# kaist-ina/BWA-MEME

Hardware: AMD Instinct MI355X
Metric: seeding_reads_per_sec (higher is better)
Workload: dtype u64; 1 GPU; learned-index seeding (rounds 1-3 + hit gather), 150 bp SE reads vs 3100 Mbp synthetic genome (fwd+rc suffix array of 6200000000 entries), index and reads resident in HBM; genome_bp=3100000000, sa_entries=6200000000, read_len=150, rmi_leaves_log2=28

## Files before the change

bwa-meme_amd/csrc/meme_seed.hip:

```cpp
#include <limits.h>
#include <stdlib.h>
#include <string.h>
#include <utility>

#include "meme_seed_kernel.h"

namespace {

using namespace seedk;

constexpr int SCAN_BLOCK = 256;
constexpr int SCAN_ITEMS = 4;
constexpr int SCAN_TILE = SCAN_BLOCK * SCAN_ITEMS;

__device__ __forceinline__ i64 block_scan_excl(i64 v, i64* total) {
    __shared__ i64 wsum[SCAN_BLOCK / 64];
    const int lane = threadIdx.x & 63, wid = threadIdx.x >> 6;
    i64 x = v;
#pragma unroll
    for (int d = 1; d < 64; d <<= 1) {
        i64 y = __shfl_up(x, d);
        if (lane >= d) x += y;
    }
    if (lane == 63) wsum[wid] = x;
// ... 103 lines not shown
            if (hits_per_smem > 0 && h > hits_per_smem) h = hits_per_smem;
            i64 incl = h;
#pragma unroll
            for (int d = 1; d < GL; d <<= 1) {
                i64 y = __shfl_up(incl, d, GL);
                if (t >= d) incl += y;
            }
            const i64 hb = hb0 + incl - h;
            u64 first = 0;
            if (act) {
                first = (s.sa_start & SLOT_POS) ? (u64)(s.sa_start & SLOT_VAL) : sa[s.sa_start].pos;
                meme_mem_tl m;
                m.start = s.start;
                m.end = s.end;
                m.hitbeg = (int32_t)hb;
                m.hitcount = s.count > (i64)INT_MAX ? INT_MAX : (int32_t)s.count;
                m.cache_refpos = first;
                out[k] = m;
                if (h > 0) hout[hb] = first;
                for (i64 i = 1; i < h && i < 4; ++i) hout[hb + i] = sa[s.sa_start + i].pos;
            }
            u64 longmask = (__ballot(act && h > 4) >> gbase) & 0xffffull;
            while (longmask) {
                const int src = __ffsll((long long)longmask) - 1;
                longmask &= longmask - 1;
                const i64 lh = __shfl(h, src, GL), lhb = __shfl(hb, src, GL), lsa = __shfl(s.sa_start, src, GL);
                for (i64 i = 4 + t; i < lh; i += GL) hout[lhb + i] = sa[lsa + i].pos;
            }
            hb0 += __shfl(incl, GL - 1, GL);
        }
    }
}

template <int G>
int launch_k_seed(hipStream_t stream, const SeedArgs& A, size_t lds, i64 blocks) {
    if (lds > 64 * 1024)
        HIP_TRY(hipFuncSetAttribute((const void*)k_seed<G>, hipFuncAttributeMaxDynamicSharedMemorySize, (int)lds));
    hipLaunchKernelGGL(k_seed<G>, dim3((unsigned)blocks), dim3(BLOCK), lds, stream, A);
    HIP_TRY(hipGetLastError());
    return MEME_OK;
}

struct SeedRun {
    meme_ctx* ctx;
    const i64* d_read_off; i64 nreads;
    const meme_seed_opt* opt;
    PackGeom geo;
    TierTable tiers = {};
    bool defer = false;
    i64 n_early = -1;
    i64 n_todo = 0;
    float ms_total = 0.f, ms_reseed = 0.f;
    i64 launches = 0, searches = 0, windows = 0, lane_searches = 0;
};

int seed_pack(SeedRun& R, const uint8_t* d_reads, i64 max_len, i64 total_bytes) {
    meme_ctx* ctx = R.ctx;
    if (max_len > MAX_READ_LEN) {
        meme_set_error("read of %lld bases exceeds the learned-index limit of %d (LEARNED_MAX_READ_LEN)", (long long)max_len, MAX_READ_LEN);
        return MEME_E_ARG;
    }
    if (max_len < 1) max_len = 1;
    PackGeom& geo = R.geo;
    geo.W = (int)((max_len + 31) / 32) + 2;
    geo.MW = (int)((max_len + 63) / 64);
    geo.stride = 2 * geo.W + 2 * geo.MW + 1;
    int rc;
    if ((rc = meme_buf_reserve(ctx, ctx->batch.packed, (size_t)R.nreads * geo.stride * 8))) return rc;
    HIP_TRY(hipEventRecord(ctx->seed.ev[SEED_EV_PACK0], ctx->stream));
    int rb = (int)((48 * 1024) / max_len);
    if (rb > 32) rb = 32;
    if (rb < 1) rb = 1;
    i64 pblocks = (R.nreads + rb - 1) / rb;
    if (pblocks > (i64)ctx->n_cus * 16) pblocks = (i64)ctx->n_cus * 16;
    size_t plds = ((size_t)rb * (size_t)max_len + 16 + 48 + 3) & ~(size_t)3;
    hipLaunchKernelGGL(k_pack_reads, dim3((unsigned)pblocks), dim3(256), plds, ctx->stream, d_reads,
                       R.d_read_off, R.nreads, total_bytes, geo, rb, (u64*)ctx->batch.packed.p);
    HIP_TRY(hipGetLastError());
    HIP_TRY(hipEventRecord(ctx->seed.ev[SEED_EV_PACK1], ctx->stream));
    return MEME_OK;
}

int launch_tier(SeedRun& R, int tier, i64 n_todo, const i64* pending, int cset, hipStream_t stream, bool defer) {
    meme_ctx* ctx = R.ctx;
    int G = tier == 0 ? (int)ctx->group_lanes : 32;
    const int cap = tier == 0 ? (int)ctx->smem_cap : TIER_CAP[tier];
    const int lcap = cap < TIER_LCAP[tier] ? cap : TIER_LCAP[tier];
    DevBuf& sb = ctx->seed.slots[tier];
    DevBuf& ob = ctx->seed.ovf[tier & 1];
    const size_t need = (size_t)n_todo * cap * sizeof(SlotRec);
    if (tier > 0 && need > sb.cap) {
        size_t free_b = 0;
        if (!meme_fits_free_hbm(need, 0, &free_b)) {
            meme_set_error("%lld reads emitted more than %d SMEMs each: re-running them needs %.1f GB of slots, more than half of the "
                           "free HBM (%.1f GB); seed this batch in smaller pieces", (long long)n_todo, R.tiers.cap[tier - 1],
                           need / 1e9, free_b / 1e9);
            return MEME_E_CAPACITY;
        }
    }
    int rc;
    if ((rc = meme_buf_reserve(ctx, sb, need))) return rc;
    if ((rc = meme_buf_reserve(ctx, ob, (size_t)n_todo * sizeof(i64)))) return rc;
    unsigned long long* counters = ctx->seed.counter_set(cset);
    HIP_TRY(hipMemsetAsync(counters, 0, SEED_CTRS * sizeof(unsigned long long), stream));
    SeedArgs A;
    A.I = ctx->idx;
    A.packed = (const u64*)ctx->batch.packed.p;
    A.read_off = R.d_read_off;
    A.nreads = n_todo;
    A.geo = R.geo;
    A.opt = *R.opt;
    A.slots = (SlotRec*)sb.p;
    A.slot_cnt = (int*)ctx->seed.slot_cnt.p;
    A.slot_hits = (i64*)ctx->seed.slot_hits.p;
    A.slot_loc = (i64*)ctx->seed.slot_loc.p;
    A.pending = pending;
    A.ovf_list = (i64*)ob.p;
    A.cap = cap;
    A.lcap = lcap;
    A.tier = tier;
    A.counters = counters;
    A.defer = defer ? 1 : 0;
    R.tiers.base[tier] = (const SlotRec*)sb.p;
    R.tiers.cap[tier] = cap;
    while (G < 32 && seed_lds_bytes(G, R.geo, lcap) > (size_t)160 * 1024) G *= 2;
    const int groups = BLOCK / G;
    size_t lds = seed_lds_bytes(G, R.geo, lcap);
    i64 want = (n_todo + groups - 1) / groups;
    i64 blocks = ctx->seed_blocks > 0 ? ctx->seed_blocks : (i64)ctx->n_cus * ctx->seed_blocks_per_cu;
    if (blocks > want) blocks = want;
    if (blocks < 1) blocks = 1;
    if (tier == 0) HIP_TRY(hipEventRecord(ctx->seed.ev[SEED_EV_SEARCH0], stream));
    switch (G) {
    case 1: return launch_k_seed<1>(stream, A, lds, blocks);
    case 2: return launch_k_seed<2>(stream, A, lds, blocks);
    case 4: return launch_k_seed<4>(stream, A, lds, blocks);
    case 8: return launch_k_seed<8>(stream, A, lds, blocks);
    case 16: return launch_k_seed<16>(stream, A, lds, blocks);
    case 32: return launch_k_seed<32>(stream, A, lds, blocks);
    default: meme_set_error("group_lanes must be 1, 2, 4, 8, 16 or 32"); return MEME_E_ARG;
    }
}

int fetch_counters(SeedRun& R, int cset, unsigned long long* h) {
    HIP_TRY(hipMemcpyAsync(h, R.ctx->seed.counter_set(cset), SEED_CTRS * sizeof(unsigned long long), hipMemcpyDeviceToHost, R.ctx->stream));
    HIP_TRY(hipStreamSynchronize(R.ctx->stream));
    return MEME_OK;
}
void tally(SeedRun& R, const unsigned long long* h) {
    ++R.launches;
    R.searches += (i64)h[SEED_CTR_SEARCHES];
    R.windows += (i64)h[SEED_CTR_WINDOWS];
    R.n_todo = (i64)h[SEED_CTR_OVERFLOW];
#ifdef SEED_PROF
    {
        double tot = 0; for (int k = 0; k < 8; ++k) tot += (double)h[SEED_CTR_PROF + k];
        fprintf(stderr, "[seed prof]:");
        const char* nm[6] = {"control", "request+rmi", "window+compare", "resolve", "level", "apply"};
        for (int k = 0; k < 6; ++k) fprintf(stderr, " %s %.1f%%", nm[k], 100.0 * (double)h[SEED_CTR_PROF + k] / (tot > 0 ? tot : 1));
        fprintf(stderr, "\n");
    }
#endif
}

int launch_reseed(SeedRun& R) {
    meme_ctx* ctx = R.ctx;
    SeedWs& S = ctx->seed;
    const i64 nreads = R.nreads;
    HIP_TRY(hipEventRecord(S.ev[SEED_EV_RESEED0], ctx->stream));
    ReseedArgs A;
    A.I = ctx->idx; A.packed = (const u64*)ctx->batch.packed.p; A.geo = R.geo; A.nreads = nreads; A.opt = *R.opt;
    A.slots = (SlotRec*)S.slots[0].p; A.cap = (int)ctx->smem_cap; A.slot_cnt = (int*)S.slot_cnt.p; A.slot_hits = (i64*)S.slot_hits.p;
    A.ovf_list = (i64*)S.ovf[0].p; A.counters = S.counter_set(0); A.pend_list = (i64*)S.pend.p;
    A.blk = (BlkRec*)S.blk.p; A.blk_out = A.blk + nreads * BLK_PER_READ; A.blk_cap = nreads * BLK_PER_READ;
    A.blk_ctr = SEED_CTR_BLK; A.blk_out_ctr = SEED_CTR_BLK_OUT;
    i64 rblocks = (nreads + 255) / 256;
    if (rblocks > (i64)ctx->n_cus * 32) rblocks = (i64)ctx->n_cus * 32;
    hipLaunchKernelGGL(k_reseed, dim3((unsigned)rblocks), dim3(256), 0, ctx->stream, A);
    HIP_TRY(hipEventRecord(ctx->side.fork[0], ctx->stream));
    const unsigned sblocks = (unsigned)(rblocks < (i64)ctx->n_cus * 4 ? rblocks : (i64)ctx->n_cus * 4);
    if (!S.emit.s) HIP_TRY(hipStreamCreateWithFlags(&S.emit.s, hipStreamNonBlocking));
    for (int i = 0; i < 2; ++i) if (!S.emit_ev[i]) HIP_TRY(hipEventCreateWithFlags(&S.emit_ev[i], hipEventDisableTiming));
    HIP_TRY(hipEventRecord(S.emit_ev[0], ctx->stream));
    HIP_TRY(hipStreamWaitEvent(S.emit, S.emit_ev[0], 0));
    hipLaunchKernelGGL(k_reseed_emit, dim3(sblocks), dim3(256), 0, S.emit, A);
    HIP_TRY(hipEventRecord(S.emit_ev[1], S.emit));
    constexpr int ROUNDS = 4;
    for (int round = 0; round < ROUNDS; ++round) {
        hipLaunchKernelGGL(k_reseed_search, dim3(sblocks), dim3(256), 0, ctx->stream, A);
        if (round < ROUNDS - 1) {
            hipLaunchKernelGGL(k_reseed_resume<false>, dim3(sblocks), dim3(256), 0, ctx->stream, A);
            HIP_TRY(hipMemsetAsync(S.counter_set(0) + A.blk_ctr, 0, sizeof(unsigned long long), ctx->stream));
            std::swap(A.blk, A.blk_out); std::swap(A.blk_ctr, A.blk_out_ctr);
        } else hipLaunchKernelGGL(k_reseed_resume<true>, dim3(sblocks), dim3(256), 0, ctx->stream, A);
    }
    HIP_TRY(hipGetLastError());
    return MEME_OK;
}

int launch_early_overflow(SeedRun& R) {
    meme_ctx* ctx = R.ctx;
    Stream& side = ctx->side.st[0];
    unsigned long long h_ovf = 0;
    HIP_TRY(hipStreamWaitEvent(side, ctx->side.fork[0], 0));
    HIP_TRY(hipMemcpyAsync(&h_ovf, ctx->seed.counter_set(0) + SEED_CTR_OVERFLOW, 8, hipMemcpyDeviceToHost, side));
    HIP_TRY(hipStreamSynchronize(side));
    if (h_ovf == 0) return MEME_OK;
    R.n_early = (i64)h_ovf;
    int rc;
    if ((rc = launch_tier(R, 1, R.n_early, (const i64*)ctx->seed.ovf[0].p, 1, side, false))) return rc;
    HIP_TRY(hipEventRecord(ctx->side.done[0], side));
    HIP_TRY(hipStreamWaitEvent(ctx->stream, ctx->side.done[0], 0));
    return MEME_OK;
}

int seed_tier0(SeedRun& R) {
    meme_ctx* ctx = R.ctx;
    SeedWs& S = ctx->seed;
    int rc;
    R.defer = ctx->seed_defer != 0 && ctx->idx.plcp != nullptr && R.opt->rounds >= 2;
    if (R.defer && (rc = meme_buf_reserve(ctx, S.pend, (size_t)R.nreads * sizeof(i64)))) return rc;
    if (R.defer && (rc = meme_buf_reserve(ctx, S.blk, (size_t)R.nreads * BLK_PER_READ * 2 * sizeof(BlkRec)))) return rc;
    if ((rc = launch_tier(R, 0, R.nreads, nullptr, 0, ctx->stream, R.defer))) return rc;
    if (R.defer) {
        if ((rc = meme_side_stream(ctx, 0)) || (rc = launch_reseed(R)) || (rc = launch_early_overflow(R))) return rc;
        HIP_TRY(hipStreamWaitEvent(ctx->stream, S.emit_ev[1], 0));
    }
    HIP_TRY(hipEventRecord(S.ev[SEED_EV_SEARCH1], ctx->stream));
    unsigned long long h[SEED_CTRS];
    if ((rc = fetch_counters(R, 0, h))) return rc;
    float ms = 0.f;
    HIP_TRY(hipEventElapsedTime(&ms, S.ev[SEED_EV_SEARCH0], S.ev[SEED_EV_SEARCH1]));
    R.ms_total += ms;
    if (R.defer) {
        float a = 0.f;
        HIP_TRY(hipEventElapsedTime(&a, S.ev[SEED_EV_RESEED0], S.ev[SEED_EV_SEARCH1]));
        R.ms_reseed += a;
        R.lane_searches += (i64)h[SEED_CTR_LANE];
        if (getenv("MEME_SEED_TRACE")) fprintf(stderr, "[meme] seed tier 0: search kernel + re-seeding kernels %.2f ms, of which behind k_seed %.2f ms (%lld lane searches; %lld reads of the "
                                               "overflow tier beside them)\n", ms, a, (long long)h[SEED_CTR_LANE], (long long)(R.n_early < 0 ? 0 : R.n_early));
    }
    tally(R, h);
    return MEME_OK;
}

int seed_overflow_tiers(SeedRun& R) {
    meme_ctx* ctx = R.ctx;
    SeedWs& S = ctx->seed;
    int rc;
    unsigned long long h[SEED_CTRS];
    for (int tier = 1; R.n_todo > 0; ++tier) {
        if (tier >= N_TIERS) {
            meme_set_error("a read produced more than %d SMEMs", TIER_CAP[N_TIERS - 1]);
            return MEME_E_CAPACITY;
        }
        const int cset = tier & 1;
        if (tier == 1 && R.n_early == R.n_todo) {
            if ((rc = fetch_counters(R, cset, h))) return rc;
        } else {
            HIP_TRY(hipEventRecord(S.ev[SEED_EV_SEARCH0], ctx->stream));
            if ((rc = launch_tier(R, tier, R.n_todo, (const i64*)S.ovf[(tier - 1) & 1].p, cset, ctx->stream, false))) return rc;
            HIP_TRY(hipEventRecord(S.ev[SEED_EV_SEARCH1], ctx->stream));
            if ((rc = fetch_counters(R, cset, h))) return rc;
            float ms = 0.f;
            HIP_TRY(hipEventElapsedTime(&ms, S.ev[SEED_EV_SEARCH0], S.ev[SEED_EV_SEARCH1]));
            R.ms_total += ms;
        }
        tally(R, h);
    }
    return MEME_OK;
}

int seed_gather(SeedRun& R, meme_seed_result* out) {
    meme_ctx* ctx = R.ctx;
    SeedWs& S = ctx->seed;
    ResidentBatch& B = ctx->batch;
    const i64 nreads = R.nreads;
    int rc;
    i64 ntiles = (nreads + SCAN_TILE - 1) / SCAN_TILE;
    if ((rc = meme_buf_reserve(ctx, ctx->scan_tmp, (size_t)(2 * ntiles + 2) * sizeof(i64)))) return rc;
    if ((rc = meme_buf_reserve(ctx, B.smem_off, (size_t)(nreads + 1) * sizeof(i64)))) return rc;
    if ((rc = meme_buf_reserve(ctx, B.hit_off, (size_t)(nreads + 1) * sizeof(i64)))) return rc;
    i64* tiles = (i64*)ctx->scan_tmp.p;
    i64* totals = tiles + 2 * ntiles;
    HIP_TRY(hipEventRecord(S.ev[SEED_EV_GATHER0], ctx->stream));
    hipLaunchKernelGGL(k_tile_sums, dim3((unsigned)ntiles), dim3(SCAN_BLOCK), 0, ctx->stream, (const int*)S.slot_cnt.p,
                       (const i64*)S.slot_hits.p, nreads, tiles);
    hipLaunchKernelGGL(k_scan_tiles, dim3(1), dim3(SCAN_BLOCK), 0, ctx->stream, tiles, ntiles, totals);
    hipLaunchKernelGGL(k_offsets, dim3((unsigned)ntiles), dim3(SCAN_BLOCK), 0, ctx->stream, (const int*)S.slot_cnt.p,
                       (const i64*)S.slot_hits.p, nreads, (const i64*)tiles, (i64*)B.smem_off.p, (i64*)B.hit_off.p);
    HIP_TRY(hipGetLastError());
    i64 h_tot[2];
    HIP_TRY(hipMemcpyAsync(h_tot, totals, sizeof(h_tot), hipMemcpyDeviceToHost, ctx->stream));
    HIP_TRY(hipStreamSynchronize(ctx->stream));
    if ((rc = meme_buf_reserve(ctx, B.smems, (size_t)(h_tot[0] + 1) * sizeof(meme_mem_tl)))) return rc;
    if ((rc = meme_buf_reserve(ctx, B.hits, (size_t)(h_tot[1] + 1) * sizeof(u64)))) return rc;
    i64 gblocks = (nreads + 15) / 16;
    if (gblocks > (i64)ctx->n_cus * 8) gblocks = (i64)ctx->n_cus * 8;
    if (gblocks < 1) gblocks = 1;
    hipLaunchKernelGGL(k_gather, dim3((unsigned)gblocks), dim3(BLOCK), 0, ctx->stream, ctx->idx.sa, R.tiers,
                       (const i64*)S.slot_loc.p, (const int*)S.slot_cnt.p, nreads, R.opt->hits_per_smem,
                       (const i64*)B.smem_off.p, (const i64*)B.hit_off.p, (meme_mem_tl*)B.smems.p, (u64*)B.hits.p);
    HIP_TRY(hipGetLastError());
    HIP_TRY(hipEventRecord(S.ev[SEED_EV_GATHER1], ctx->stream));
    HIP_TRY(hipStreamSynchronize(ctx->stream));
    HIP_TRY(hipEventElapsedTime(&ctx->tm.seed_gather_ms, S.ev[SEED_EV_GATHER0], S.ev[SEED_EV_GATHER1]));
    out->d_smems = (const meme_mem_tl*)B.smems.p;
    out->d_smem_off = (const i64*)B.smem_off.p;
    out->d_hits = (const u64*)B.hits.p;
    out->d_hit_off = (const i64*)B.hit_off.p;
    out->total_smems = h_tot[0];
// ... 250 lines not shown
```

bwa-meme_amd/csrc/meme_seed_kernel.h:

```cpp
#pragma once
#include <limits.h>

#include "meme_common.h"

namespace seedk {

constexpr int BLOCK = 256;
constexpr int MAX_READ_LEN = 500;

struct SlotRec {
    int32_t start, end;
    i64 sa_start;
    i64 count;
};
constexpr i64 SLOT_POS = 1ll << 62;
constexpr i64 SLOT_DEFER = 1ll << 61;
constexpr i64 SLOT_PEND = 1ll << 59;
constexpr i64 SLOT_VAL = (1ll << 48) - 1;
constexpr int DEFER_MAX_K = 64;


constexpr int N_TIERS = 3;
constexpr int TIER_CAP[N_TIERS] = {64, 2048, 65536};
#ifndef LCAP0
// ... 819 lines not shown


__device__ __forceinline__ u64 ext_g(const u64* __restrict__ w, int s) {
    const int k = s >> 5, sh = (s & 31) * 2;
    const u64 a = w[k], b = w[k + 1];
    return sh ? (a << sh) | (b >> (64 - sh)) : a;
}

struct LaneQuery {
    const u64* s;
    int off, vlen;
    u64 wq;
};

__device__ __forceinline__ void lane_compare_ent(const DevIndex& I, const LaneQuery& q, int cap, const SaEnt e, int& lcp, bool& less) {
    const i64 nlimit = I.n - (i64)cap;
    int Lc = cap;
    if ((i64)e.pos > nlimit) Lc = (int)(I.n - (i64)e.pos);
    const u64 x = e.key ^ q.wq;
    bool lt = e.key < q.wq;
    int l = x ? (__clzll((long long)x) >> 1) : 32;
    if (!x && 32 < Lc) {
        const i64 p0 = (i64)e.pos + 32;
        for (int k = 1;; ++k) {
            const u64 wr = extract32(I.pac, p0 + 32 * (k - 1));
            const u64 qq = ext_g(q.s, q.off + 32 * k);
            const u64 y = wr ^ qq;
            if (y) { l += __clzll((long long)y) >> 1; lt = wr < qq; break; }
            l += 32;
            if (l >= Lc) break;
        }
    }
    if (l >= Lc) { lcp = Lc; less = (i64)e.pos < nlimit; }
    else { lcp = l; less = lt; }
}
__device__ __forceinline__ void lane_compare(const DevIndex& I, const LaneQuery& q, int cap, i64 slot, int& lcp, bool& less) {
    lane_compare_ent(I, q, cap, I.sa[slot], lcp, less);
}

constexpr int LANE_W = 16;
struct LaneWin {
    uint32_t* lw;
    i64 base;
    __device__ __forceinline__ bool has(i64 slot) const { return base >= 0 && slot >= base && slot < base + LANE_W; }
    __device__ __forceinline__ int get(i64 slot) const { const int i = (int)(slot - base); return (int)((lw[(i >> 1) * 256] >> (16 * (i & 1))) & 0xffffu); }
};
__device__ __forceinline__ int lane_lcp(const DevIndex& I, const LaneQuery& q, const LaneWin& C, int cap, i64 slot) {
    if (C.has(slot)) return C.get(slot);
    int lc; bool ls;
    lane_compare(I, q, cap, slot, lc, ls);
    return lc;
}

__device__ __forceinline__ void lane_search(const DevIndex& I, const LaneQuery& q, int min_intv, uint32_t* lw, int& r_L, i64& r_start, i64& r_count) {
    const i64 n = I.n;
    u64 key = q.wq;
    if (q.vlen < 32) key |= (~0ull) >> (2 * q.vlen);
    u64 err;
    const i64 p = rmi_lookup((glb_rmi)I.l2, (glb_rmi)I.l1, I.n_l1, I.shift, n, key, err);
    LaneWin C; C.lw = lw; C.base = -1;
    int L = 0;
    i64 s = 0, e = 0;
    bool located = false;
    int lc; bool ls;
    {
        const i64 below = (i64)((err >> 32) & 0x3fffffffull) + 1, above = (i64)(err & 0x7fffffffull);
        const i64 span = below + above + 1;
        i64 base = span <= LANE_W ? p - below - (LANE_W - span) / 2 : p - (below * LANE_W) / span;
        if (base < 0) base = 0;
        if (base > n - LANE_W) base = n - LANE_W;
        SaEnt ent[LANE_W];
#pragma unroll
        for (int k = 0; k < LANE_W; ++k) ent[k] = I.sa[base + k];
        unsigned lessm = 0;
        int prev = 0;
#pragma unroll
        for (int k = 0; k < LANE_W; ++k) {
            lane_compare_ent(I, q, q.vlen, ent[k], lc, ls);
            lessm |= (ls ? 1u : 0u) << k;
            if (k & 1) lw[(k >> 1) * 256] = (uint32_t)prev | ((uint32_t)lc << 16); else prev = lc;
        }
        C.base = base;
        const int P = __popc(lessm);
        if (lessm == ((1u << P) - 1u) && ((P > 0 && P < LANE_W) || (P == 0 && base == 0) || (P == LANE_W && base + LANE_W == n))) {
            const int lm = P > 0 ? C.get(base + P - 1) : -1, lp = P < LANE_W ? C.get(base + P) : -1;
            L = lm >= lp ? lm : lp;
            s = e = base + (lm >= lp ? P - 1 : P);
            located = true;
        }
    }
    if (!located) {
        i64 lo = -1, hi = n;
        lane_compare(I, q, q.vlen, p, lc, ls);
        if (ls) {
            lo = p;
            for (i64 st = 1; hi == n && lo < n - 1; st <<= 1) {
                i64 pr = lo + st; if (pr > n - 1) pr = n - 1;
                lane_compare(I, q, q.vlen, pr, lc, ls);
                if (ls) lo = pr; else hi = pr;
            }
        } else {
            hi = p;
            for (i64 st = 1; lo == -1 && hi > 0; st <<= 1) {
                i64 pr = hi - st; if (pr < 0) pr = 0;
                lane_compare(I, q, q.vlen, pr, lc, ls);
                if (ls) lo = pr; else hi = pr;
            }
        }
        while (hi - lo > 1) {
            const i64 mid = lo + (hi - lo) / 2;
            lane_compare(I, q, q.vlen, mid, lc, ls);
            if (ls) lo = mid; else hi = mid;
        }
        const i64 P = hi;
        const int lm = P > 0 ? lane_lcp(I, q, C, q.vlen, P - 1) : -1, lp = P < n ? lane_lcp(I, q, C, q.vlen, P) : -1;
        L = lm >= lp ? lm : lp;
        s = e = lm >= lp ? P - 1 : P;
    }
    for (;;) {
        while (s > 0 && C.has(s - 1) && C.get(s - 1) >= L) --s;
        if (s > 0 && !C.has(s - 1)) {
            i64 good = s, bad = -1;
            for (i64 st = 1; good > 0; st <<= 1) {
                i64 pr = good - st; if (pr < 0) pr = 0;
                if (lane_lcp(I, q, C, L, pr) >= L) good = pr; else { bad = pr; break; }
            }
            while (bad >= 0 && good - bad > 1) {
                const i64 mid = bad + (good - bad) / 2;
                if (lane_lcp(I, q, C, L, mid) >= L) good = mid; else bad = mid;
            }
            s = good;
        }
        while (e < n - 1 && C.has(e + 1) && C.get(e + 1) >= L) ++e;
        if (e < n - 1 && !C.has(e + 1)) {
            i64 good = e, bad = n;
// ... 85 lines not shown
    }
};

struct RegionState { int pivot, next, guard, stage; };

template <bool OWNED>
__device__ __forceinline__ bool region_walk(const PlcpView& V, i64 n, i64 T0, int qbeg, int qend, int l_seq, int msl, RegionState& S, unsigned& hops,
                                            SmemAppender<OWNED>& ap, int& n_pend) {
    for (;;) {
        if (S.stage == 0) {
            const int plc = V.fwd(T0 + S.pivot);
            if (plc == 0 || plc == 255 || plc >= qend - S.pivot) return true;
            ++hops; S.next = S.pivot + plc; S.stage = 1;
        }
        if (S.stage == 1) {
            if (S.pivot >= S.next || ++S.guard > 4 * l_seq + 16) { S.stage = 3; return false; }
            const int plc = (S.pivot >= qbeg && S.pivot < qend) ? V.rev(n - 1 - (T0 + S.pivot)) : 0;
            if (plc == 0 || plc == 255 || plc >= S.pivot - qbeg + 1) return true;
            ++hops; S.pivot = S.pivot - plc + 1;
            if (S.next - S.pivot < msl) { S.stage = 3; return false; }
            S.stage = 2;
        }
        const int plc = (S.pivot >= qbeg && S.pivot < qend) ? V.fwd(T0 + S.pivot) : 0;
        if (plc == 0 || plc == 255 || plc >= qend - S.pivot) return true;
        if (plc >= msl) {
            if (!OWNED) return true;
            ap.push(S.pivot, S.pivot + plc, SLOT_PEND, 0);
            ++n_pend;
        }
        ++hops; S.pivot = S.pivot + plc; S.stage = 1;
    }
}

__device__ __forceinline__ LaneQuery region_query(const u64* __restrict__ rec, const PackGeom& geo, int l_seq, bool has_n, const RegionState& S) {
    LaneQuery q;
    const bool left = S.stage == 1;
    q.s = rec + (left ? geo.W : 0);
    q.off = left ? l_seq - 1 - S.pivot : S.pivot;
    q.vlen = first_n_g(rec + 2 * geo.W + (left ? geo.MW : 0), has_n, q.off, l_seq) - q.off;
    q.wq = ext_g(q.s, q.off);
    return q;
}

template <bool OWNED>
__device__ __forceinline__ void region_apply(RegionState& S, int msl, int r_L, i64 r_start, i64 r_count, SmemAppender<OWNED>& ap) {
    if (S.stage == 0) { S.next = S.pivot + r_L; S.stage = 1; }
    else if (S.stage == 1) { S.pivot = S.pivot - r_L + 1; S.stage = (S.next - S.pivot < msl) ? 3 : 2; }
    else {
        if (r_L >= msl) ap.push(S.pivot, S.pivot + r_L, r_start, r_count);
        S.pivot = S.pivot + r_L; S.stage = 1;
    }
}

__device__ __forceinline__ void stage_plcp_windows(const uint8_t* __restrict__ plcp, const PlcpView& V, uint32_t* win) {
    uint4 v[2 * (PLCP_WIN / 16)];
#pragma unroll
    for (int q = 0; q < PLCP_WIN / 16; ++q) {
        v[q] = *reinterpret_cast<const uint4*>(plcp + V.F0 + 16 * q);
        v[PLCP_WIN / 16 + q] = *reinterpret_cast<const uint4*>(plcp + V.R0 + 16 * q);
    }
#pragma unroll
    for (int q = 0; q < 2 * (PLCP_WIN / 16); ++q) {
        win[(4 * q + 0) * 256] = v[q].x; win[(4 * q + 1) * 256] = v[q].y; win[(4 * q + 2) * 256] = v[q].z; win[(4 * q + 3) * 256] = v[q].w;
    }
}

constexpr int BLK_PER_READ = 1;
constexpr int BLK_MORE = 16;

__global__ void __launch_bounds__(256) k_reseed(ReseedArgs A) {
    __shared__ uint32_t win[2 * (PLCP_WIN / 4) * 256];
    __shared__ unsigned long long blk_hops, blk_lane;
    __shared__ unsigned blk_pend, blk_pend_base, blk_blk;
    __shared__ unsigned long long blk_blk_base;
    const uint8_t* __restrict__ plcp = A.I.plcp;
    const i64 n = A.I.n;
    const int msl = A.opt.min_seed_len, cap = A.cap;
    for (i64 r0 = (i64)blockIdx.x * blockDim.x; r0 < A.nreads; r0 += (i64)gridDim.x * blockDim.x) {
        if (threadIdx.x == 0) { blk_hops = 0; blk_lane = 0; blk_pend = 0; blk_blk = 0; }
        __syncthreads();
        const i64 r = r0 + threadIdx.x;
        unsigned hops = 0, lsearches = 0;
        int n_pend = 0, n_blk = 0, pend_ns = 0;
        BlkRec held[BLK_PER_READ];
        if (r < A.nreads) {
            const int c0 = A.slot_cnt[r];
            const int c = c0 > DEFER_MAX_K ? DEFER_MAX_K : c0;
            SlotRec* sl = A.slots + r * cap;
            const u64* rec = A.packed + r * A.geo.stride;
            SmemAppender<true> ap;
            ap.sl = sl; ap.cap = cap; ap.hps = A.opt.hits_per_smem; ap.ns = c0; ap.hits_add = 0; ap.rid = r;
            int l_seq = 0;
            int k = -1;
            for (;;) {
                i64 f = 0;
                for (++k; k < c; ++k) { f = sl[k].sa_start; if (f & SLOT_DEFER) break; }
                if (k >= c) break;
                if (l_seq == 0) { const u64 lw = rec[A.geo.stride - 1]; l_seq = (int)(lw & 0x7fffffffull); }
                const int qbeg = sl[k].start, qend = sl[k].end;
                const i64 T0 = (f & SLOT_VAL) - qbeg;
                PlcpView V;
                V.plcp = plcp; V.win = win + threadIdx.x;
                RegionState S;
                S.pivot = (qbeg + qend) >> 1; S.next = 0; S.guard = 0; S.stage = 0;
                V.F0 = plcp_win_fwd(T0, S.pivot); V.R0 = plcp_win_rev(T0, S.pivot, n);
                stage_plcp_windows(plcp, V, win + threadIdx.x);
                if (region_walk<true>(V, n, T0, qbeg, qend, l_seq, msl, S, hops, ap, n_pend)) {
                    BlkRec b;
                    b.rid = r; b.k = k; b.pivot = S.pivot; b.next = S.next; b.guard = S.guard; b.r_L = 0; b.r_start = 0; b.r_count = 0;
                    b.stage = S.stage | (n_blk == BLK_PER_READ - 1 ? BLK_MORE : 0);
#pragma unroll
                    for (int i = 0; i < BLK_PER_READ; ++i) if (i == n_blk) held[i] = b;
                    if (++n_blk == BLK_PER_READ) break;
                }
            }
            if (ap.ns != c0) {
                if (ap.ns > cap) {
                    A.slot_cnt[r] = 0; A.slot_hits[r] = 0;
                    A.ovf_list[atomicAdd(&A.counters[SEED_CTR_OVERFLOW], 1ull)] = r;
                    n_pend = 0; n_blk = 0;
                } else { A.slot_cnt[r] = ap.ns; A.slot_hits[r] = A.slot_hits[r] + ap.hits_add; pend_ns = ap.ns; }
            }
        }
        unsigned my_pend = 0, my_blk = 0;
        if (n_pend) my_pend = atomicAdd(&blk_pend, 1u);
        if (n_blk) my_blk = atomicAdd(&blk_blk, (unsigned)n_blk);
        if (hops | lsearches) { atomicAdd(&blk_hops, (unsigned long long)(hops + lsearches)); if (lsearches) atomicAdd(&blk_lane, (unsigned long long)lsearches); }
        __syncthreads();
        if (threadIdx.x == 0) {
            if (blk_hops) atomicAdd(&A.counters[SEED_CTR_SEARCHES], blk_hops);
            if (blk_lane) atomicAdd(&A.counters[SEED_CTR_LANE], blk_lane);
            if (blk_pend) blk_pend_base = (unsigned)atomicAdd(&A.counters[SEED_CTR_PEND], (unsigned long long)blk_pend);
            if (blk_blk) blk_blk_base = atomicAdd(&A.counters[A.blk_ctr], (unsigned long long)blk_blk);
        }
        __syncthreads();
        if (n_pend) A.pend_list[blk_pend_base + my_pend] = r | ((i64)pend_ns << 40);
#pragma unroll
        for (int i = 0; i < BLK_PER_READ; ++i)
            if (i < n_blk) {
                const unsigned long long at = blk_blk_base + my_blk + i;
                if ((i64)at < A.blk_cap) A.blk[at] = held[i];
            }
        __syncthreads();
    }
}

__global__ void __launch_bounds__(256) k_reseed_emit(ReseedArgs A) {
    __shared__ uint32_t lwin[(LANE_W / 2) * 256];
    const i64 n_list = (i64)A.counters[SEED_CTR_PEND];
    for (i64 i = (i64)blockIdx.x * blockDim.x + threadIdx.x; i < n_list; i += (i64)gridDim.x * blockDim.x) {
        const i64 ent = A.pend_list[i];
        const i64 r = ent & ((1ll << 40) - 1);
        const int c = (int)(ent >> 40);
        SlotRec* sl = A.slots + r * A.cap;
        const u64* rec = A.packed + r * A.geo.stride;
        i64 hits_add = 0;
        int k = -1;
        for (;;) {
            for (++k; k < c; ++k) if (sl[k].sa_start & SLOT_PEND) break;
            if (k >= c) break;
            LaneQuery q;
            q.s = rec; q.off = sl[k].start; q.vlen = sl[k].end - sl[k].start;
            q.wq = ext_g(q.s, q.off);
            int r_L; i64 r_start, r_count;
            lane_search(A.I, q, 1, lwin + threadIdx.x, r_L, r_start, r_count);
            sl[k].sa_start = r_start; sl[k].count = r_count;
            hits_add += (A.opt.hits_per_smem > 0 && r_count > A.opt.hits_per_smem) ? (i64)A.opt.hits_per_smem : r_count;
        }
        atomicAdd(reinterpret_cast<unsigned long long*>(A.slot_hits + r), (unsigned long long)hits_add);
    }
}

__global__ void __launch_bounds__(256) k_reseed_search(ReseedArgs A) {
    __shared__ uint32_t lwin[(LANE_W / 2) * 256];
    i64 n_blk = (i64)A.counters[A.blk_ctr];
    if (n_blk > A.blk_cap) n_blk = A.blk_cap;
    for (i64 i = (i64)blockIdx.x * blockDim.x + threadIdx.x; i < n_blk; i += (i64)gridDim.x * blockDim.x) {
        BlkRec b = A.blk[i];
        const u64* rec = A.packed + b.rid * A.geo.stride;
        const u64 lw = rec[A.geo.stride - 1];
        RegionState S;
        S.pivot = b.pivot; S.next = b.next; S.guard = b.guard; S.stage = b.stage & ~BLK_MORE;
        const LaneQuery q = region_query(rec, A.geo, (int)(lw & 0x7fffffffull), ((lw >> 31) & 1ull) != 0, S);
        lane_search(A.I, q, 2, lwin + threadIdx.x, b.r_L, b.r_start, b.r_count);
        A.blk[i].r_L = b.r_L; A.blk[i].r_start = b.r_start; A.blk[i].r_count = b.r_count;
    }
}

template <bool LAST>
__global__ void __launch_bounds__(256) k_reseed_resume(ReseedArgs A) {
    __shared__ uint32_t win[2 * (PLCP_WIN / 4) * 256];
    __shared__ uint32_t lwin[(LANE_W / 2) * 256];
    __shared__ unsigned long long acc_total, acc_lane, out_base;
    __shared__ unsigned out_n;
    const uint8_t* __restrict__ plcp = A.I.plcp;
    const i64 n = A.I.n;
    const int msl = A.opt.min_seed_len;
    if (threadIdx.x == 0) { acc_total = 0; acc_lane = 0; }
    i64 n_blk = (i64)A.counters[A.blk_ctr];
    if (n_blk > A.blk_cap) n_blk = A.blk_cap;
    unsigned total = 0, lsearches = 0;
    for (i64 i0 = (i64)blockIdx.x * blockDim.x; i0 < n_blk; i0 += (i64)gridDim.x * blockDim.x) {
        if (threadIdx.x == 0) out_n = 0;
        __syncthreads();
        const i64 i = i0 + threadIdx.x;
        bool blocked = false;
        BlkRec nb;
        if (i < n_blk) {
            const BlkRec b = A.blk[i];
            const i64 r = b.rid;
            SlotRec* sl = A.slots + r * A.cap;
            const u64* rec = A.packed + r * A.geo.stride;
            const u64 lw = rec[A.geo.stride - 1];
            const int l_seq = (int)(lw & 0x7fffffffull);
            const bool has_n = ((lw >> 31) & 1ull) != 0;
            SmemAppender<false> ap;
            ap.sl = sl; ap.cap = A.cap; ap.cnt = A.slot_cnt + r; ap.hits = A.slot_hits + r; ap.ovf_list = A.ovf_list; ap.counters = A.counters; ap.rid = r;
            ap.hps = A.opt.hits_per_smem; ap.ns = 0; ap.hits_add = 0;
            unsigned hops = 1;
            int k = b.k;
            const int c = (b.stage & BLK_MORE) ? (A.slot_cnt[r] > DEFER_MAX_K ? DEFER_MAX_K : A.slot_cnt[r]) : 0;
            bool first = true;
            for (;;) {
                const int qbeg = sl[k].start, qend = sl[k].end;
                const i64 T0 = (sl[k].sa_start & SLOT_VAL) - qbeg;
                PlcpView V;
                V.plcp = plcp; V.win = win + threadIdx.x;
                V.F0 = plcp_win_fwd(T0, (qbeg + qend) >> 1); V.R0 = plcp_win_rev(T0, (qbeg + qend) >> 1, n);
                stage_plcp_windows(plcp, V, win + threadIdx.x);
                RegionState S;
                if (first) {
                    S.pivot = b.pivot; S.next = b.next; S.guard = b.guard; S.stage = b.stage & ~BLK_MORE;
                    region_apply<false>(S, msl, b.r_L, b.r_start, b.r_count, ap);
                    first = false;
                } else { S.pivot = (qbeg + qend) >> 1; S.next = 0; S.guard = 0; S.stage = 0; }
                while (S.stage != 3) {
                    int n_pend = 0;
                    if (!region_walk<false>(V, n, T0, qbeg, qend, l_seq, msl, S, hops, ap, n_pend)) break;
                    if (!LAST) {
                        nb.rid = r; nb.k = k; nb.pivot = S.pivot; nb.next = S.next; nb.guard = S.guard; nb.stage = S.stage | (b.stage & BLK_MORE);
                        nb.r_L = 0; nb.r_start = 0; nb.r_count = 0;
                        blocked = true;
                        break;
                    }
                    const LaneQuery q = region_query(rec, A.geo, l_seq, has_n, S);
                    int r_L; i64 r_start, r_count;
                    lane_search(A.I, q, 2, lwin + threadIdx.x, r_L, r_start, r_count);
                    ++lsearches; ++hops;
                    region_apply<false>(S, msl, r_L, r_start, r_count, ap);
                }
                if (blocked) break;
                for (++k; k < c; ++k) if ((sl[k].sa_start & (SLOT_DEFER | SLOT_POS)) == (SLOT_DEFER | SLOT_POS)) break;
                if (k >= c) break;
            }
            total += hops;
        }
        unsigned my = 0;
        if (blocked) my = atomicAdd(&out_n, 1u);
        __syncthreads();
        if (threadIdx.x == 0 && out_n) out_base = atomicAdd(&A.counters[A.blk_out_ctr], (unsigned long long)out_n);
        __syncthreads();
        if (blocked) A.blk_out[out_base + my] = nb;
        __syncthreads();
    }
    if (total) atomicAdd(&acc_total, (unsigned long long)total);
    if (lsearches) atomicAdd(&acc_lane, (unsigned long long)lsearches);
    __syncthreads();
    if (threadIdx.x == 0) {
        if (acc_total) atomicAdd(&A.counters[SEED_CTR_SEARCHES], acc_total);
        if (acc_lane) atomicAdd(&A.counters[SEED_CTR_LANE], acc_lane);
    }
}

}
```

Before: 150.2 million reads/s.

## Cooperate in quads for SA window and PLCP loads in re-seeding kernels

Restructures lane_search and stage_plcp_windows so the four lanes of a quad load each other's SA window and PLCP windows together, broadcasting base addresses with DPP. The per-lane strided scattered loads become coalesced quad-wide loads. The re-seeding kernels are made wave-convergent (all lanes loop until __any is false) so the cross-lane ops stay valid. This adds idle-lane work and divergence costs. It also merges the early overflow counter fetch into the tier-0 readback, saving a sync, and sets an occupancy launch bound on k_reseed_resume.

```diff
diff --git a/bwa-meme_amd/csrc/meme_seed.hip b/bwa-meme_amd/csrc/meme_seed.hip
--- a/bwa-meme_amd/csrc/meme_seed.hip
+++ b/bwa-meme_amd/csrc/meme_seed.hip
@@ -179,6 +179,7 @@
     i64 n_todo = 0;
     float ms_total = 0.f, ms_reseed = 0.f;
     i64 launches = 0, searches = 0, windows = 0, lane_searches = 0;
+    unsigned long long h_early[SEED_CTRS];
 };
 
 int seed_pack(SeedRun& R, const uint8_t* d_reads, i64 max_len, i64 total_bytes) {
@@ -269,8 +270,8 @@
     }
 }
 
-int fetch_counters(SeedRun& R, int cset, unsigned long long* h) {
-    HIP_TRY(hipMemcpyAsync(h, R.ctx->seed.counter_set(cset), SEED_CTRS * sizeof(unsigned long long), hipMemcpyDeviceToHost, R.ctx->stream));
+int fetch_counters(SeedRun& R, int cset, unsigned long long* h, int nsets = 1) {
+    HIP_TRY(hipMemcpyAsync(h, R.ctx->seed.counter_set(cset), (size_t)nsets * SEED_CTRS * sizeof(unsigned long long), hipMemcpyDeviceToHost, R.ctx->stream));
     HIP_TRY(hipStreamSynchronize(R.ctx->stream));
     return MEME_OK;
 }
@@ -354,8 +355,9 @@
         HIP_TRY(hipStreamWaitEvent(ctx->stream, S.emit_ev[1], 0));
     }
     HIP_TRY(hipEventRecord(S.ev[SEED_EV_SEARCH1], ctx->stream));
-    unsigned long long h[SEED_CTRS];
-    if ((rc = fetch_counters(R, 0, h))) return rc;
+    unsigned long long h[2 * SEED_CTRS];
+    if ((rc = fetch_counters(R, 0, h, R.n_early >= 0 ? 2 : 1))) return rc;
+    if (R.n_early >= 0) memcpy(R.h_early, h + SEED_CTRS, sizeof(R.h_early));
     float ms = 0.f;
     HIP_TRY(hipEventElapsedTime(&ms, S.ev[SEED_EV_SEARCH0], S.ev[SEED_EV_SEARCH1]));
     R.ms_total += ms;
@@ -383,7 +385,7 @@
         }
         const int cset = tier & 1;
         if (tier == 1 && R.n_early == R.n_todo) {
-            if ((rc = fetch_counters(R, cset, h))) return rc;
+            memcpy(h, R.h_early, sizeof(h));
         } else {
             HIP_TRY(hipEventRecord(S.ev[SEED_EV_SEARCH0], ctx->stream));
             if ((rc = launch_tier(R, tier, R.n_todo, (const i64*)S.ovf[(tier - 1) & 1].p, cset, ctx->stream, false))) return rc;
diff --git a/bwa-meme_amd/csrc/meme_seed_kernel.h b/bwa-meme_amd/csrc/meme_seed_kernel.h
--- a/bwa-meme_amd/csrc/meme_seed_kernel.h
+++ b/bwa-meme_amd/csrc/meme_seed_kernel.h
@@ -895,35 +895,75 @@
     return lc;
 }
 
-__device__ __forceinline__ void lane_search(const DevIndex& I, const LaneQuery& q, int min_intv, uint32_t* lw, int& r_L, i64& r_start, i64& r_count) {
+template <int J> __device__ __forceinline__ int quad_bcast(int v) { return __builtin_amdgcn_update_dpp(0, v, J * 0x55, 0xF, 0xF, true); }
+template <int J> __device__ __forceinline__ u64 quad_bcast64(u64 v) {
+    return ((u64)(unsigned)quad_bcast<J>((int)(v >> 32)) << 32) | (u64)(unsigned)quad_bcast<J>((int)(unsigned)v);
+}
+__device__ __forceinline__ void lds_handoff() {
+    __builtin_amdgcn_fence(__ATOMIC_RELEASE, "wavefront"); __builtin_amdgcn_wave_barrier(); __builtin_amdgcn_fence(__ATOMIC_ACQUIRE, "wavefront");
+}
+template <int J>
+__device__ __forceinline__ void quad_window_load(const SaEnt* __restrict__ sa, i64 base, int t, SaEnt (&ent)[LANE_W / 4]) {
+    const i64 bo = (i64)quad_bcast64<J>((u64)base);
+#pragma unroll
+    for (int i = 0; i < LANE_W / 4; ++i) ent[i] = sa[bo + 4 * i + t];
+}
+template <int J>
+__device__ __forceinline__ unsigned quad_window_compare(const DevIndex& I, const LaneQuery& q, bool active, int t, const SaEnt (&ent)[LANE_W / 4], uint32_t* lwq) {
+    LaneQuery qo;
+    qo.s = reinterpret_cast<const u64*>(quad_bcast64<J>((u64)reinterpret_cast<uintptr_t>(q.s)));
+    const int ov = quad_bcast<J>(q.off | (q.vlen << 16));
+    qo.off = ov & 0xffff; qo.vlen = (int)((unsigned)ov >> 16);
+    qo.wq = quad_bcast64<J>(q.wq);
+    const bool ao = quad_bcast<J>(active ? 1 : 0) != 0;
+    unsigned m = 0;
+    if (ao) {
+        unsigned short* col = reinterpret_cast<unsigned short*>(lwq + J) + (t & 1);
+#pragma unroll
+        for (int i = 0; i < LANE_W / 4; ++i) {
+            int lc; bool ls;
+            lane_compare_ent(I, qo, qo.vlen, ent[i], lc, ls);
+            m |= (ls ? 1u : 0u) << (4 * i + t);
+            col[(2 * i + (t >> 1)) * 512] = (unsigned short)lc;
+        }
+    }
+    return (unsigned)group_or<4>((int)m);
+}
+
+__device__ __forceinline__ void lane_search(const DevIndex& I, const LaneQuery& q, bool active, int min_intv, uint32_t* lw, int& r_L, i64& r_start, i64& r_count) {
     const i64 n = I.n;
-    u64 key = q.wq;
-    if (q.vlen < 32) key |= (~0ull) >> (2 * q.vlen);
-    u64 err;
-    const i64 p = rmi_lookup((glb_rmi)I.l2, (glb_rmi)I.l1, I.n_l1, I.shift, n, key, err);
-    LaneWin C; C.lw = lw; C.base = -1;
+    const int t = threadIdx.x & 3;
+    i64 p = 0, base = 0;
+    if (active) {
+        u64 key = q.wq;
+        if (q.vlen < 32) key |= (~0ull) >> (2 * q.vlen);
+        u64 err;
+        p = rmi_lookup((glb_rmi)I.l2, (glb_rmi)I.l1, I.n_l1, I.shift, n, key, err);
+        const i64 below = (i64)((err >> 32) & 0x3fffffffull) + 1, above = (i64)(err & 0x7fffffffull);
+        const i64 span = below + above + 1;
+        base = span <= LANE_W ? p - below - (LANE_W - span) / 2 : p - (below * LANE_W) / span;
+        if (base < 0) base = 0;
+        if (base > n - LANE_W) base = n - LANE_W;
+    }
+    unsigned lessm;
+    {
+        lds_handoff();
+        SaEnt e0[LANE_W / 4], e1[LANE_W / 4], e2[LANE_W / 4], e3[LANE_W / 4];
+        quad_window_load<0>(I.sa, base, t, e0); quad_window_load<1>(I.sa, base, t, e1);
+        quad_window_load<2>(I.sa, base, t, e2); quad_window_load<3>(I.sa, base, t, e3);
+        uint32_t* lwq = lw - t;
+        const unsigned m0 = quad_window_compare<0>(I, q, active, t, e0, lwq), m1 = quad_window_compare<1>(I, q, active, t, e1, lwq);
+        const unsigned m2 = quad_window_compare<2>(I, q, active, t, e2, lwq), m3 = quad_window_compare<3>(I, q, active, t, e3, lwq);
+        lessm = t == 0 ? m0 : (t == 1 ? m1 : (t == 2 ? m2 : m3));
+        lds_handoff();
+    }
+    if (!active) return;
+    LaneWin C; C.lw = lw; C.base = base;
     int L = 0;
     i64 s = 0, e = 0;
     bool located = false;
     int lc; bool ls;
     {
-        const i64 below = (i64)((err >> 32) & 0x3fffffffull) + 1, above = (i64)(err & 0x7fffffffull);
-        const i64 span = below + above + 1;
-        i64 base = span <= LANE_W ? p - below - (LANE_W - span) / 2 : p - (below * LANE_W) / span;
-        if (base < 0) base = 0;
-        if (base > n - LANE_W) base = n - LANE_W;
-        SaEnt ent[LANE_W];
-#pragma unroll
-        for (int k = 0; k < LANE_W; ++k) ent[k] = I.sa[base + k];
-        unsigned lessm = 0;
-        int prev = 0;
-#pragma unroll
-        for (int k = 0; k < LANE_W; ++k) {
-            lane_compare_ent(I, q, q.vlen, ent[k], lc, ls);
-            lessm |= (ls ? 1u : 0u) << k;
-            if (k & 1) lw[(k >> 1) * 256] = (uint32_t)prev | ((uint32_t)lc << 16); else prev = lc;
-        }
-        C.base = base;
         const int P = __popc(lessm);
         if (lessm == ((1u << P) - 1u) && ((P > 0 && P < LANE_W) || (P == 0 && base == 0) || (P == LANE_W && base + LANE_W == n))) {
             const int lm = P > 0 ? C.get(base + P - 1) : -1, lp = P < LANE_W ? C.get(base + P) : -1;
@@ -1115,17 +1155,31 @@
     }
 }
 
-__device__ __forceinline__ void stage_plcp_windows(const uint8_t* __restrict__ plcp, const PlcpView& V, uint32_t* win) {
-    uint4 v[2 * (PLCP_WIN / 16)];
-#pragma unroll
-    for (int q = 0; q < PLCP_WIN / 16; ++q) {
-        v[q] = *reinterpret_cast<const uint4*>(plcp + V.F0 + 16 * q);
-        v[PLCP_WIN / 16 + q] = *reinterpret_cast<const uint4*>(plcp + V.R0 + 16 * q);
-    }
-#pragma unroll
-    for (int q = 0; q < 2 * (PLCP_WIN / 16); ++q) {
-        win[(4 * q + 0) * 256] = v[q].x; win[(4 * q + 1) * 256] = v[q].y; win[(4 * q + 2) * 256] = v[q].z; win[(4 * q + 3) * 256] = v[q].w;
-    }
+template <int J>
+__device__ __forceinline__ void quad_plcp_load(const uint8_t* __restrict__ plcp, i64 F0, i64 R0, int t, uint4& vf, uint4& vr) {
+    vf = *reinterpret_cast<const uint4*>(plcp + (i64)quad_bcast64<J>((u64)F0) + 16 * t);
+    vr = *reinterpret_cast<const uint4*>(plcp + (i64)quad_bcast64<J>((u64)R0) + 16 * t);
+}
+template <int J>
+__device__ __forceinline__ void quad_plcp_store(bool active, int t, const uint4& vf, const uint4& vr, uint32_t* winq) {
+    if (quad_bcast<J>(active ? 1 : 0) == 0) return;
+    uint32_t* f = winq + J + (4 * t) * 256;
+    uint32_t* r = f + (PLCP_WIN / 4) * 256;
+    f[0] = vf.x; f[256] = vf.y; f[512] = vf.z; f[768] = vf.w;
+    r[0] = vr.x; r[256] = vr.y; r[512] = vr.z; r[768] = vr.w;
+}
+__device__ __forceinline__ void stage_plcp_windows(const uint8_t* __restrict__ plcp, i64 F0, i64 R0, bool active, uint32_t* win) {
+    static_assert(PLCP_WIN == 64, "four 16-byte pieces per window, one per quad lane");
+    const int t = threadIdx.x & 3;
+    if (!active) { F0 = 0; R0 = 0; }
+    lds_handoff();
+    uint4 vf[4], vr[4];
+    quad_plcp_load<0>(plcp, F0, R0, t, vf[0], vr[0]); quad_plcp_load<1>(plcp, F0, R0, t, vf[1], vr[1]);
+    quad_plcp_load<2>(plcp, F0, R0, t, vf[2], vr[2]); quad_plcp_load<3>(plcp, F0, R0, t, vf[3], vr[3]);
+    uint32_t* winq = win - t;
+    quad_plcp_store<0>(active, t, vf[0], vr[0], winq); quad_plcp_store<1>(active, t, vf[1], vr[1], winq);
+    quad_plcp_store<2>(active, t, vf[2], vr[2], winq); quad_plcp_store<3>(active, t, vf[3], vr[3], winq);
+    lds_handoff();
 }
 
 constexpr int BLK_PER_READ = 1;
@@ -1146,38 +1200,48 @@
         unsigned hops = 0, lsearches = 0;
         int n_pend = 0, n_blk = 0, pend_ns = 0;
         BlkRec held[BLK_PER_READ];
-        if (r < A.nreads) {
-            const int c0 = A.slot_cnt[r];
+        {
+            const bool have = r < A.nreads;
+            const int c0 = have ? A.slot_cnt[r] : 0;
             const int c = c0 > DEFER_MAX_K ? DEFER_MAX_K : c0;
-            SlotRec* sl = A.slots + r * cap;
-            const u64* rec = A.packed + r * A.geo.stride;
+            SlotRec* sl = A.slots + (have ? r : 0) * cap;
+            const u64* rec = A.packed + (have ? r : 0) * A.geo.stride;
             SmemAppender<true> ap;
             ap.sl = sl; ap.cap = cap; ap.hps = A.opt.hits_per_smem; ap.ns = c0; ap.hits_add = 0; ap.rid = r;
             int l_seq = 0;
             int k = -1;
+            bool live = have;
             for (;;) {
                 i64 f = 0;
-                for (++k; k < c; ++k) { f = sl[k].sa_start; if (f & SLOT_DEFER) break; }
-                if (k >= c) break;
-                if (l_seq == 0) { const u64 lw = rec[A.geo.stride - 1]; l_seq = (int)(lw & 0x7fffffffull); }
-                const int qbeg = sl[k].start, qend = sl[k].end;
-                const i64 T0 = (f & SLOT_VAL) - qbeg;
+                if (live) {
+                    for (++k; k < c; ++k) { f = sl[k].sa_start; if (f & SLOT_DEFER) break; }
+                    if (k >= c) live = false;
+                }
+                if (!__any(live)) break;
+                int qbeg = 0, qend = 0;
+                i64 T0 = 0;
                 PlcpView V;
-                V.plcp = plcp; V.win = win + threadIdx.x;
+                V.plcp = plcp; V.win = win + threadIdx.x; V.F0 = 0; V.R0 = 0;
                 RegionState S;
-                S.pivot = (qbeg + qend) >> 1; S.next = 0; S.guard = 0; S.stage = 0;
-                V.F0 = plcp_win_fwd(T0, S.pivot); V.R0 = plcp_win_rev(T0, S.pivot, n);
-                stage_plcp_windows(plcp, V, win + threadIdx.x);
-                if (region_walk<true>(V, n, T0, qbeg, qend, l_seq, msl, S, hops, ap, n_pend)) {
+                S.pivot = 0; S.next = 0; S.guard = 0; S.stage = 0;
+                if (live) {
+                    if (l_seq == 0) { const u64 lw = rec[A.geo.stride - 1]; l_seq = (int)(lw & 0x7fffffffull); }
+                    qbeg = sl[k].start; qend = sl[k].end;
+                    T0 = (f & SLOT_VAL) - qbeg;
+                    S.pivot = (qbeg + qend) >> 1;
+                    V.F0 = plcp_win_fwd(T0, S.pivot); V.R0 = plcp_win_rev(T0, S.pivot, n);
+                }
+                stage_plcp_windows(plcp, V.F0, V.R0, live, win + threadIdx.x);
+                if (live && region_walk<true>(V, n, T0, qbeg, qend, l_seq, msl, S, hops, ap, n_pend)) {
                     BlkRec b;
                     b.rid = r; b.k = k; b.pivot = S.pivot; b.next = S.next; b.guard = S.guard; b.r_L = 0; b.r_start = 0; b.r_count = 0;
                     b.stage = S.stage | (n_blk == BLK_PER_READ - 1 ? BLK_MORE : 0);
 #pragma unroll
                     for (int i = 0; i < BLK_PER_READ; ++i) if (i == n_blk) held[i] = b;
-                    if (++n_blk == BLK_PER_READ) break;
-                }
-            }
-            if (ap.ns != c0) {
+                    if (++n_blk == BLK_PER_READ) live = false;
+                }
+            }
+            if (have && ap.ns != c0) {
                 if (ap.ns > cap) {
                     A.slot_cnt[r] = 0; A.slot_hits[r] = 0;
                     A.ovf_list[atomicAdd(&A.counters[SEED_CTR_OVERFLOW], 1ull)] = r;
@@ -1211,26 +1275,37 @@
 __global__ void __launch_bounds__(256) k_reseed_emit(ReseedArgs A) {
     __shared__ uint32_t lwin[(LANE_W / 2) * 256];
     const i64 n_list = (i64)A.counters[SEED_CTR_PEND];
-    for (i64 i = (i64)blockIdx.x * blockDim.x + threadIdx.x; i < n_list; i += (i64)gridDim.x * blockDim.x) {
-        const i64 ent = A.pend_list[i];
+    for (i64 i0 = (i64)blockIdx.x * blockDim.x; i0 < n_list; i0 += (i64)gridDim.x * blockDim.x) {
+        const i64 i = i0 + threadIdx.x;
+        const bool have = i < n_list;
+        const i64 ent = have ? A.pend_list[i] : 0;
         const i64 r = ent & ((1ll << 40) - 1);
         const int c = (int)(ent >> 40);
         SlotRec* sl = A.slots + r * A.cap;
         const u64* rec = A.packed + r * A.geo.stride;
         i64 hits_add = 0;
         int k = -1;
+        bool live = have;
         for (;;) {
-            for (++k; k < c; ++k) if (sl[k].sa_start & SLOT_PEND) break;
-            if (k >= c) break;
+            if (live) {
+                for (++k; k < c; ++k) if (sl[k].sa_start & SLOT_PEND) break;
+                if (k >= c) live = false;
+            }
+            if (!__any(live)) break;
             LaneQuery q;
-            q.s = rec; q.off = sl[k].start; q.vlen = sl[k].end - sl[k].start;
-            q.wq = ext_g(q.s, q.off);
-            int r_L; i64 r_start, r_count;
-            lane_search(A.I, q, 1, lwin + threadIdx.x, r_L, r_start, r_count);
-            sl[k].sa_start = r_start; sl[k].count = r_count;
-            hits_add += (A.opt.hits_per_smem > 0 && r_count > A.opt.hits_per_smem) ? (i64)A.opt.hits_per_smem : r_count;
-        }
-        atomicAdd(reinterpret_cast<unsigned long long*>(A.slot_hits + r), (unsigned long long)hits_add);
+            q.s = rec; q.off = 0; q.vlen = 0; q.wq = 0;
+            if (live) {
+                q.off = sl[k].start; q.vlen = sl[k].end - sl[k].start;
+                q.wq = ext_g(q.s, q.off);
+            }
+            int r_L = 0; i64 r_start = 0, r_count = 0;
+            lane_search(A.I, q, live, 1, lwin + threadIdx.x, r_L, r_start, r_count);
+            if (live) {
+                sl[k].sa_start = r_start; sl[k].count = r_count;
+                hits_add += (A.opt.hits_per_smem > 0 && r_count > A.opt.hits_per_smem) ? (i64)A.opt.hits_per_smem : r_count;
+            }
+        }
+        if (have) atomicAdd(reinterpret_cast<unsigned long long*>(A.slot_hits + r), (unsigned long long)hits_add);
     }
 }
 
@@ -1238,20 +1313,27 @@
     __shared__ uint32_t lwin[(LANE_W / 2) * 256];
     i64 n_blk = (i64)A.counters[A.blk_ctr];
     if (n_blk > A.blk_cap) n_blk = A.blk_cap;
-    for (i64 i = (i64)blockIdx.x * blockDim.x + threadIdx.x; i < n_blk; i += (i64)gridDim.x * blockDim.x) {
-        BlkRec b = A.blk[i];
-        const u64* rec = A.packed + b.rid * A.geo.stride;
-        const u64 lw = rec[A.geo.stride - 1];
-        RegionState S;
-        S.pivot = b.pivot; S.next = b.next; S.guard = b.guard; S.stage = b.stage & ~BLK_MORE;
-        const LaneQuery q = region_query(rec, A.geo, (int)(lw & 0x7fffffffull), ((lw >> 31) & 1ull) != 0, S);
-        lane_search(A.I, q, 2, lwin + threadIdx.x, b.r_L, b.r_start, b.r_count);
-        A.blk[i].r_L = b.r_L; A.blk[i].r_start = b.r_start; A.blk[i].r_count = b.r_count;
+    for (i64 i0 = (i64)blockIdx.x * blockDim.x; i0 < n_blk; i0 += (i64)gridDim.x * blockDim.x) {
+        const i64 i = i0 + threadIdx.x;
+        const bool have = i < n_blk;
+        LaneQuery q;
+        q.s = A.packed; q.off = 0; q.vlen = 0; q.wq = 0;
+        if (have) {
+            const BlkRec b = A.blk[i];
+            const u64* rec = A.packed + b.rid * A.geo.stride;
+            const u64 lw = rec[A.geo.stride - 1];
+            RegionState S;
+            S.pivot = b.pivot; S.next = b.next; S.guard = b.guard; S.stage = b.stage & ~BLK_MORE;
+            q = region_query(rec, A.geo, (int)(lw & 0x7fffffffull), ((lw >> 31) & 1ull) != 0, S);
+        }
+        int r_L = 0; i64 r_start = 0, r_count = 0;
+        lane_search(A.I, q, have, 2, lwin + threadIdx.x, r_L, r_start, r_count);
+        if (have) { A.blk[i].r_L = r_L; A.blk[i].r_start = r_start; A.blk[i].r_count = r_count; }
     }
 }
 
 template <bool LAST>
-__global__ void __launch_bounds__(256) k_reseed_resume(ReseedArgs A) {
+__global__ void __launch_bounds__(256, 3) k_reseed_resume(ReseedArgs A) {
     __shared__ uint32_t win[2 * (PLCP_WIN / 4) * 256];
     __shared__ uint32_t lwin[(LANE_W / 2) * 256];
     __shared__ unsigned long long acc_total, acc_lane, out_base;
@@ -1269,12 +1351,15 @@
         const i64 i = i0 + threadIdx.x;
         bool blocked = false;
         BlkRec nb;
-        if (i < n_blk) {
-            const BlkRec b = A.blk[i];
+        {
+            const bool have = i < n_blk;
+            BlkRec b;
+            b.rid = 0; b.k = 0; b.pivot = 0; b.next = 0; b.guard = 0; b.stage = 0; b.r_L = 0; b.r_start = 0; b.r_count = 0;
+            if (have) b = A.blk[i];
             const i64 r = b.rid;
             SlotRec* sl = A.slots + r * A.cap;
             const u64* rec = A.packed + r * A.geo.stride;
-            const u64 lw = rec[A.geo.stride - 1];
+            const u64 lw = have ? rec[A.geo.stride - 1] : 0;
             const int l_seq = (int)(lw & 0x7fffffffull);
             const bool has_n = ((lw >> 31) & 1ull) != 0;
             SmemAppender<false> ap;
@@ -1282,41 +1367,60 @@
             ap.hps = A.opt.hits_per_smem; ap.ns = 0; ap.hits_add = 0;
             unsigned hops = 1;
             int k = b.k;
-            const int c = (b.stage & BLK_MORE) ? (A.slot_cnt[r] > DEFER_MAX_K ? DEFER_MAX_K : A.slot_cnt[r]) : 0;
+            const int c = (have && (b.stage & BLK_MORE)) ? (A.slot_cnt[r] > DEFER_MAX_K ? DEFER_MAX_K : A.slot_cnt[r]) : 0;
             bool first = true;
-            for (;;) {
-                const int qbeg = sl[k].start, qend = sl[k].end;
-                const i64 T0 = (sl[k].sa_start & SLOT_VAL) - qbeg;
+            bool live = have;
+            while (__any(live)) {
+                int qbeg = 0, qend = 0;
+                i64 T0 = 0;
                 PlcpView V;
-                V.plcp = plcp; V.win = win + threadIdx.x;
-                V.F0 = plcp_win_fwd(T0, (qbeg + qend) >> 1); V.R0 = plcp_win_rev(T0, (qbeg + qend) >> 1, n);
-                stage_plcp_windows(plcp, V, win + threadIdx.x);
+                V.plcp = plcp; V.win = win + threadIdx.x; V.F0 = 0; V.R0 = 0;
+                if (live) {
+                    qbeg = sl[k].start; qend = sl[k].end;
+                    T0 = (sl[k].sa_start & SLOT_VAL) - qbeg;
+                    V.F0 = plcp_win_fwd(T0, (qbeg + qend) >> 1); V.R0 = plcp_win_rev(T0, (qbeg + qend) >> 1, n);
+                }
+                stage_plcp_windows(plcp, V.F0, V.R0, live, win + threadIdx.x);
                 RegionState S;
-                if (first) {
+                S.pivot = (qbeg + qend) >> 1; S.next = 0; S.guard = 0; S.stage = 0;
+                if (live && first) {
                     S.pivot = b.pivot; S.next = b.next; S.guard = b.guard; S.stage = b.stage & ~BLK_MORE;
                     region_apply<false>(S, msl, b.r_L, b.r_start, b.r_count, ap);
                     first = false;
-                } else { S.pivot = (qbeg + qend) >> 1; S.next = 0; S.guard = 0; S.stage = 0; }
-                while (S.stage != 3) {
-                    int n_pend = 0;
-                    if (!region_walk<false>(V, n, T0, qbeg, qend, l_seq, msl, S, hops, ap, n_pend)) break;
-                    if (!LAST) {
-                        nb.rid = r; nb.k = k; nb.pivot = S.pivot; nb.next = S.next; nb.guard = S.guard; nb.stage = S.stage | (b.stage & BLK_MORE);
-                        nb.r_L = 0; nb.r_start = 0; nb.r_count = 0;
-                        blocked = true;
-                        break;
-                    }
-                    const LaneQuery q = region_query(rec, A.geo, l_seq, has_n, S);
-                    int r_L; i64 r_start, r_count;
-                    lane_search(A.I, q, 2, lwin + threadIdx.x, r_L, r_start, r_count);
-                    ++lsearches; ++hops;
-                    region_apply<false>(S, msl, r_L, r_start, r_count, ap);
-                }
-                if (blocked) break;
-                for (++k; k < c; ++k) if ((sl[k].sa_start & (SLOT_DEFER | SLOT_POS)) == (SLOT_DEFER | SLOT_POS)) break;
-                if (k >= c) break;
-            }
-            total += hops;
+                }
+                bool walking = live;
+                for (;;) {
+                    bool need = false;
+                    if (walking) {
+                        int n_pend = 0;
+                        if (S.stage == 3 || !region_walk<false>(V, n, T0, qbeg, qend, l_seq, msl, S, hops, ap, n_pend)) walking = false;
+                        else if (!LAST) {
+                            nb.rid = r; nb.k = k; nb.pivot = S.pivot; nb.next = S.next; nb.guard = S.guard; nb.stage = S.stage | (b.stage & BLK_MORE);
+                            nb.r_L = 0; nb.r_start = 0; nb.r_count = 0;
+                            blocked = true;
+                            walking = false;
+                        } else need = true;
+                    }
+                    if (!LAST || !__any(need)) break;
+                    LaneQuery q;
+                    q.s = rec; q.off = 0; q.vlen = 0; q.wq = 0;
+                    if (need) q = region_query(rec, A.geo, l_seq, has_n, S);
+                    int r_L = 0; i64 r_start = 0, r_count = 0;
+                    lane_search(A.I, q, need, 2, lwin + threadIdx.x, r_L, r_start, r_count);
+                    if (need) {
+                        ++lsearches; ++hops;
+                        region_apply<false>(S, msl, r_L, r_start, r_count, ap);
+                    }
+                }
+                if (live) {
+                    if (blocked) live = false;
+                    else {
+                        for (++k; k < c; ++k) if ((sl[k].sa_start & (SLOT_DEFER | SLOT_POS)) == (SLOT_DEFER | SLOT_POS)) break;
+                        if (k >= c) live = false;
+                    }
+                }
+            }
+            if (have) total += hops;
         }
         unsigned my = 0;
         if (blocked) my = atomicAdd(&out_n, 1u);
```

Measured after the change: 153.0 million reads/s (median of 6 runs). 1.02x the previous value.
